# mako443/Text2Pos-CVPR2022

Hardware: AMD Instinct MI355X
Metric: cells+queries encoded/sec and top-k retrieval QPS, 256-pt cells, 12k-cell DB (higher is better)
Workload: dtype f16x3 (fp32 operands split hi+lo into fp16, 3 f16 MFMAs, fp32 accumulate; fp32-class error) for the encoders / f64 MFMA for the ranking

## Files before the change

include/t2p.h:

```cpp
#ifndef T2P_H
#define T2P_H
#include <stddef.h>
#include <stdint.h>

#ifdef __cplusplus
extern "C" {
#endif

#define T2P_ABI_VERSION 32
#define T2P_DEFAULT_CHUNK_OBJECTS 65000
#define T2P_MAX_CHUNK_OBJECTS 65535
#define T2P_TUNING_MASK 0xD
#define T2P_E_ARG (-1)
#define T2P_E_WORKSPACE (-2)
#define T2P_E_UNSUPPORTED (-3)

typedef void* t2p_stream_t;

int t2p_abi_version(void);
const char* t2p_last_error(void);

typedef struct t2p_cell_weights {
    const float* sa_w1[3];
    const float* sa_b1[3];
// ... 230 lines not shown
int t2p_hardest_ranking(const float* scores, int32_t batch, float margin, float* best, int32_t* where, float* d_scores,
                        t2p_stream_t stream);

int t2p_sample_group(const float* xyz, int64_t n_obj, int32_t n_pts, const float* radius_host ,
                     uint8_t* const* fps_idx , uint8_t* const* nbr , uint8_t* const* cnt ,
                     t2p_stream_t stream);
int t2p_group_rows(const float* xyz, int64_t n_obj, int32_t n_pts, const float* radius_host , int32_t self_loops,
                   uint8_t* const* fps_idx , uint16_t* const* rows , uint16_t* const* n_rows ,
                   t2p_stream_t stream);
int t2p_group_rows_shared(const float* xyz, int64_t n_obj, int32_t n_pts, const float* radius_host , int32_t self_loops,
                          int32_t share_mask, uint8_t* const* fps_idx , uint16_t* const* rows ,
                          uint16_t* const* n_rows , t2p_stream_t stream);
int t2p_group_rows_built(const float* xyz, const float* rgb, int64_t n_obj, int32_t n_pts, const float* radius_host ,
                         int32_t self_loops, int32_t share_mask, uint8_t* const* fps_idx , uint16_t* const* rows ,
                         uint16_t* const* n_rows , t2p_stream_t stream);
int t2p_edge_counts(const uint16_t* rows, const uint16_t* n_rows, const int32_t* first_obj, int64_t n_obj, int32_t n_dense,
                    int32_t n_cent, int32_t self_loops, int32_t* counts, t2p_stream_t stream);
int t2p_edge_expand(const uint16_t* rows, const uint16_t* n_rows, const int32_t* first_obj, const int32_t* cent_ptr, int64_t n_obj,
                    int32_t n_dense, int32_t n_cent, int32_t self_loops, int32_t* src, int32_t* dst, t2p_stream_t stream);
int t2p_dedup_rows(const float* xyz, const float* rgb, int64_t n_obj, int32_t n_pts, uint16_t* rows, uint16_t* n_rows,
                   t2p_stream_t stream);
int t2p_knn(const float* x, int32_t dim, const int32_t* seg_ptr, int32_t n_seg, int32_t max_seg_rows, int32_t k,
            int32_t* out_idx, t2p_stream_t stream);
int t2p_gemm(const float* a, int32_t lda, const float* w, const float* bias, float* c, int32_t ldc, int32_t c0,
             int64_t m, int32_t k, int32_t n, int32_t relu, t2p_stream_t stream);
int t2p_gemm_residual(const float* a, int32_t lda, const float* w, const float* bias, float* c, int32_t ldc, int32_t c0,
                      int64_t m, int32_t k, int32_t n, int32_t relu, const float* resid, int32_t ldr, t2p_stream_t stream);
int t2p_gemm_x3(const float* a, int32_t lda, const void* wx, float scale, const float* bias, float* c, int32_t ldc, int32_t c0,
                int64_t m, int32_t k, int32_t n, int32_t relu, const float* resid, int32_t ldr, uint32_t* amax_in,
                t2p_stream_t stream);
// ... 15 lines not shown
```

profiles/tail_rows_census.py:

```python
#!/usr/bin/env python
import argparse
import os
import sys

import numpy as np

sys.path.insert(0, os.path.join(os.path.dirname(os.path.abspath(__file__)), ".."))

RADII = (0.2, 0.3, 0.4)
MAX_NBR = 32


def level(pos: np.ndarray, r: float):
    n_d = pos.shape[0]
    n_c = (n_d + 1) // 2
    r2 = np.float32(r) * np.float32(r)
    mind = np.full(n_d, np.inf, dtype=np.float32)
    fps = np.zeros(n_c, dtype=np.int64)
    cnt = np.zeros(n_c, dtype=np.int64)
    cur = 0
    for c in range(n_c):
        fps[c] = cur
        d = pos - pos[cur]
        d2 = (d[:, 0] * d[:, 0] + d[:, 1] * d[:, 1]) + d[:, 2] * d[:, 2]
        cnt[c] = min(int((d2 < r2).sum()), MAX_NBR)
        mind = np.minimum(mind, d2)
        cur = int(np.argmax(mind))
    return fps, cnt


def dedup_hits(pos: np.ndarray, rgb: np.ndarray, fps: np.ndarray, r: float) -> int:
    key = np.concatenate([pos, rgb], axis=1).view(np.uint32)
    _, first = np.unique(key, axis=0, return_index=True)
    orig = np.zeros(pos.shape[0], dtype=bool)
    orig[first] = True
    r2 = np.float32(r) * np.float32(r)
    kept = 0
    for c in fps:
        d = pos - pos[c]
        d2 = (d[:, 0] * d[:, 0] + d[:, 1] * d[:, 1]) + d[:, 2] * d[:, 2]
        hits = np.flatnonzero(d2 < r2)[:MAX_NBR]
        kept += int(orig[hits].sum())
    return kept
# ... 3 lines not shown
    ap = argparse.ArgumentParser(description=__doc__.split("\n")[0])
    ap.add_argument("--seed", type=int, default=20220002, help="bench.py's object stream")
    ap.add_argument("--objects", type=int, default=3000)
    args = ap.parse_args()
    from importlib import import_module
    S = import_module("text2pos-cvpr2022_amd.synthetic")
    xyz, rgb, _, _ = S.make_objects(args.seed, 0, args.objects)
    n = xyz.shape[0]
    rows = np.zeros(3)
    rows_dedup = 0.0
    with_tail = np.zeros(3)
    tail_cent = np.zeros(3)
    tail_rows = np.zeros(3)
    executed = np.zeros(3)
    cents = np.zeros(3)
    for o in range(n):
        pos = xyz[o].astype(np.float32)
        for l in range(3):
            fps, cnt = level(pos, RADII[l])
            n_c = fps.shape[0]
            tail = (fps == 0) & (np.arange(n_c) > 0)
            all_rows = cnt.sum() + n_c
            t_rows = cnt[tail].sum()
            rows[l] += all_rows
            cents[l] += n_c
            with_tail[l] += tail.any()
            tail_cent[l] += tail.sum()
            tail_rows[l] += t_rows
            executed[l] += all_rows - t_rows + (cnt[0] if tail.any() else 0)
            if l == 0:
                rows_dedup += dedup_hits(pos, rgb[o].astype(np.float32), fps, RADII[0]) + n_c
            pos = pos[fps]
    print(f"{n} objects of seed {args.seed}")
    print("level | rows/object | objects with a tail | tail centroids | tail rows (non-self) | rows/object, tail shared")
    for l in range(3):
        extra = f" ({rows_dedup / n:.0f} after point dedup)" if l == 0 else ""
        print(f"SA{l + 1}   | {rows[l] / n:8.0f}{extra} | {100 * with_tail[l] / n:5.1f} % | {100 * tail_cent[l] / cents[l]:5.1f} % | "
              f"{100 * tail_rows[l] / rows[l]:5.1f} % | {executed[l] / n:8.0f} ({100 * (executed[l] / rows[l] - 1):+.1f} %)")


if __name__ == "__main__":
    main()
```

text2pos-cvpr2022_amd/_lib.py:

```python
import ctypes as C
import os

import torch

_HERE = os.path.dirname(os.path.abspath(__file__))
LIB_PATH = os.environ.get("T2P_LIB") or os.path.join(_HERE, "libt2p_hip.so")
ABI_VERSION = 32

c_float_p = C.POINTER(C.c_float)
c_void = C.c_void_p


class CellWeights(C.Structure):
    _names = (["sa_w1", "sa_b1", "sa_w2", "sa_b2"], ["ga_w1", "ga_b1", "ga_w2", "ga_b2", "lin1_w", "lin1_b", "lin2_w",
              "lin2_b", "pn_w", "pn_b", "col_w1", "col_b1", "col_w2", "col_b2", "pos_w1", "pos_b1", "pos_w2", "pos_b2",
              "merge_w", "merge_b", "g_wp", "g_bp", "g_wq", "g_w2", "g_b2", "lin_w1", "lin_b1", "lin_w2", "lin_b2"])
    _fields_ = ([(n, c_void * 3) for n in _names[0]] + [(n, c_void) for n in _names[1]] +
                [("sa_w2_x3", c_void * 3), ("ga_w2_x3", c_void), ("sa_b2_x3", c_void * 3), ("sa_w2_scale", C.c_float * 3),
                 ("lin1_x3", c_void), ("lin2_x3", c_void), ("merge_x3", c_void), ("pn_x3", c_void), ("g_wp_x3", c_void),
                 ("g_wq_x3", c_void), ("lin1_scale", C.c_float), ("lin2_scale", C.c_float), ("merge_scale", C.c_float),
                 ("pn_scale", C.c_float), ("g_wp_scale", C.c_float), ("g_wq_scale", C.c_float),
                 ("sa_w1_x3", c_void * 3), ("ga_w1_x3", c_void),
                 ("class_embedding", c_void), ("color_embedding", c_void),
                 ("ga_w1_l1", C.c_float), ("ga_b1_absmax", C.c_float), ("sa_wp_l1", C.c_float * 3),
# ... 94 lines not shown
    "t2p_matching_loss_backward": (C.c_int, [c_void, C.c_int64, C.c_int32, C.c_int32, c_void, c_void, C.c_int64, c_void, c_void,
                                             c_void]),
    "t2p_mse_loss_backward": (C.c_int, [c_void, c_void, C.c_int64, c_void, c_void, c_void]),
    "t2p_colsum": (C.c_int, [c_void, C.c_int64, C.c_int32, c_void, c_void]),
    "t2p_profile_enable": (None, [C.c_int]),
    "t2p_profile_report": (C.c_int, [C.c_char_p, C.c_size_t]),
    "t2p_profile_repeat": (None, [C.c_char_p, C.c_int32]),
    "t2p_sample_group": (C.c_int, [c_void, C.c_int64, C.c_int32, c_float_p, C.POINTER(c_void), C.POINTER(c_void),
                                   C.POINTER(c_void), c_void]),
    "t2p_group_rows": (C.c_int, [c_void, C.c_int64, C.c_int32, c_float_p, C.c_int32, C.POINTER(c_void), C.POINTER(c_void),
                                 C.POINTER(c_void), c_void]),
    "t2p_group_rows_shared": (C.c_int, [c_void, C.c_int64, C.c_int32, c_float_p, C.c_int32, C.c_int32, C.POINTER(c_void),
                                        C.POINTER(c_void), C.POINTER(c_void), c_void]),
    "t2p_group_rows_built": (C.c_int, [c_void, c_void, C.c_int64, C.c_int32, c_float_p, C.c_int32, C.c_int32, C.POINTER(c_void),
                                       C.POINTER(c_void), C.POINTER(c_void), c_void]),
    "t2p_edge_counts": (C.c_int, [c_void, c_void, c_void, C.c_int64, C.c_int32, C.c_int32, C.c_int32, c_void, c_void]),
    "t2p_edge_expand": (C.c_int, [c_void, c_void, c_void, c_void, C.c_int64, C.c_int32, C.c_int32, C.c_int32, c_void, c_void, c_void]),
    "t2p_dedup_rows": (C.c_int, [c_void, c_void, C.c_int64, C.c_int32, c_void, c_void, c_void]),
    "t2p_knn": (C.c_int, [c_void, C.c_int32, c_void, C.c_int32, C.c_int32, C.c_int32, c_void, c_void]),
    "t2p_gemm": (C.c_int, [c_void, C.c_int32, c_void, c_void, c_void, C.c_int32, C.c_int32, C.c_int64, C.c_int32,
                           C.c_int32, C.c_int32, c_void]),
    "t2p_rownorm": (C.c_int, [c_void, C.c_int64, C.c_int32, c_void, c_void]),
    "t2p_gemm_residual": (C.c_int, [c_void, C.c_int32, c_void, c_void, c_void, C.c_int32, C.c_int32, C.c_int64, C.c_int32,
                                    C.c_int32, C.c_int32, c_void, C.c_int32, c_void]),
    "t2p_gemm_x3": (C.c_int, [c_void, C.c_int32, c_void, C.c_float, c_void, c_void, C.c_int32, C.c_int32, C.c_int64, C.c_int32,
                              C.c_int32, C.c_int32, c_void, C.c_int32, c_void, c_void]),
    "t2p_gemm_skinny": (C.c_int, [c_void, C.c_int32, c_void, c_void, C.c_int32, C.c_int64, C.c_int32, C.c_int32, c_void]),
    "t2p_linear_wgrad_workspace_bytes": (C.c_size_t, [C.c_int64, C.c_int32, C.c_int32]),
    "t2p_linear_wgrad_f32": (C.c_int, [c_void, C.c_int32, c_void, C.c_int32, c_void, C.c_int32, c_void, C.c_int64, C.c_int32,
                                       C.c_int32, c_void, C.c_size_t, c_void]),
# ... 34 lines not shown
```

text2pos-cvpr2022_amd/csrc/cell_encoder.hip:

```cpp
#include "../../include/t2p.h"
#include "t2p_common.h"

namespace t2p {
namespace {

struct Geo {
    int nd[3], nc[3];
    int gp;
    static constexpr int H[3] = {32, 128, 256};
    static constexpr int C[3] = {64, 128, 256};
    static constexpr int LD[3] = {96, 160, 288};
    explicit Geo(int n_pts) {
        nd[0] = n_pts;
        for (int l = 0; l < 3; l++) {
            nc[l] = (nd[l] + 1) / 2;
            if (l < 2) nd[l + 1] = nc[l];
        }
        gp = 1;
        while (gp < nc[2]) gp *= 2;
    }
    bool specialised(int l) const {
        static constexpr int ND[3] = {256, 128, 64}, NC[3] = {128, 64, 32};
        return nd[l] == ND[l] && nc[l] == NC[l];
    }
// ... 176 lines not shown
    for (int l = 0; l < 3; l++) {
        bp[l].n_rows = gt.n_rows[l];
        bp[l].n_obj = n;
        bp[l].prefix_ws = ws.prefix[l];
        bp[l].bounds_ws = ws.bounds[l];
        bp[l].W_x3 = f16x3() ? W.sa_w2_x3[l] : nullptr;
        bp[l].wp = lds_btab(l) ? W.sa_w1[l] : nullptr;
        bp[l].n_dense = g.nd[l];
        bp[l].n_cent = g.nc[l];
    }
    bp[0].w1 = sa1_points() ? W.sa_w1[0] : nullptr;
    for (int l = 0; l < 3; l++) gt.share_tail[l] = sa_shares_tail_rows(l, Geo::H[l], Geo::C[l], bp[l], cfg.n_pts, cfg.tuning) ? 1 : 0;

    const bool prune_l0 = !(cfg.tuning & 1) && cfg.n_pts == 256;
    gt.mask_l0 = prune_l0 && !(cfg.tuning & 8) && !want_nbr && gt.rows[0] && gt.rows[1] && gt.rows[2] ? 1 : 0;
    T2P_TRY(launch_sample_group(xyz, n, cfg.n_pts, cfg.radius, gt, st));
    if (gt.mask_l0)
        T2P_TRY(launch_build_rows(xyz, rgb, gt.fps_idx[0], n, cfg.n_pts, gt.rows[0], gt.n_rows[0], gt.self_loops, st));
    else if (prune_l0)
        T2P_TRY(launch_dedup_rows(xyz, rgb, n, cfg.n_pts, gt.rows[0], gt.n_rows[0], g.nc[0], st));
    return launch_sa_balance_levels(bp, Geo::H, Geo::C, st);
}

int Chunk::sa_levels(const float* xyz, const float* rgb) const {
    for (int l = 0; l < 3; l++) {
        const int H = Geo::H[l], C = Geo::C[l];
        const int cf = l == 0 ? 3 : Geo::C[l - 1];
        if (l != 0) {
            WsParams p{};
            p.A = ws.F[l - 1];
            p.lda = Geo::LD[l - 1];
            p.k_live = Geo::C[l - 1] + 4;
            p.W = W.sa_w1[l];
// ... 227 lines not shown
        gt.n_dense[l] = g.nd[l];
        gt.n_cent[l] = g.nc[l];
        gt.share_tail[l] = (share_mask >> l) & 1;
    }
    return 0;
}

int group_rows(const char* what, const float* xyz, int64_t n_obj, int32_t n_pts, const float* radius_host, int32_t self_loops,
               int32_t share_mask, uint8_t* const* fps_idx, uint16_t* const* rows, uint16_t* const* n_rows, t2p_stream_t stream) {
    T2P_CHECK_ARG(xyz && radius_host && fps_idx && rows && n_rows, "%s: NULL argument", what);
    T2P_CHECK_ARG((share_mask & ~2) == 0, "%s: share_mask=%#x (bit 1: SA level 2; no other level has a shared form)", what, share_mask);
    T2P_CHECK_ARG(share_mask == 0 || n_pts == 256, "%s: shared lists exist for 256 points per object (n_pts = %d)", what, n_pts);
    GroupTables gt;
    T2P_TRY(fill_group_tables(what, gt, n_pts, self_loops, share_mask, fps_idx, rows, n_rows, nullptr, nullptr));
    return launch_sample_group(xyz, n_obj, n_pts, radius_host, gt, (hipStream_t)stream);
}

}
}

using namespace t2p;

extern "C" {

size_t t2p_encode_cells_workspace_bytes(int64_t n_obj, int64_t n_cells, const t2p_cell_config* cfg) {
    if (cfg == nullptr || n_obj <= 0) return 256;
    int64_t n = default_chunk(*cfg);
    if (n > n_obj) n = n_obj;
    int64_t nb = n_cells < n ? n_cells : n;
    Bump b{nullptr, 0, 0};
// ... 132 lines not shown

int t2p_group_rows(const float* xyz, int64_t n_obj, int32_t n_pts, const float* radius_host, int32_t self_loops,
                   uint8_t* const* fps_idx, uint16_t* const* rows, uint16_t* const* n_rows, t2p_stream_t stream) {
    return group_rows("group_rows", xyz, n_obj, n_pts, radius_host, self_loops, 0, fps_idx, rows, n_rows, stream);
}

int t2p_group_rows_shared(const float* xyz, int64_t n_obj, int32_t n_pts, const float* radius_host, int32_t self_loops,
                          int32_t share_mask, uint8_t* const* fps_idx, uint16_t* const* rows, uint16_t* const* n_rows,
                          t2p_stream_t stream) {
    return group_rows("group_rows_shared", xyz, n_obj, n_pts, radius_host, self_loops, share_mask, fps_idx, rows, n_rows, stream);
}

int t2p_group_rows_built(const float* xyz, const float* rgb, int64_t n_obj, int32_t n_pts, const float* radius_host,
                         int32_t self_loops, int32_t share_mask, uint8_t* const* fps_idx, uint16_t* const* rows,
                         uint16_t* const* n_rows, t2p_stream_t stream) {
    T2P_CHECK_ARG(xyz && rgb && radius_host && fps_idx && rows && n_rows, "group_rows_built: NULL argument");
    T2P_CHECK_ARG(n_obj >= 0, "group_rows_built: negative size");
    T2P_CHECK_ARG((share_mask & ~2) == 0, "group_rows_built: share_mask=%#x (bit 1: SA level 2; no other level has a shared form)", share_mask);
    T2P_CHECK_ARG(n_pts == 256, "group_rows_built: built for 256 points per object (n_pts = %d)", n_pts);
    GroupTables gt;
    T2P_TRY(fill_group_tables("group_rows_built", gt, n_pts, self_loops, share_mask, fps_idx, rows, n_rows, nullptr, nullptr));
    gt.mask_l0 = 1;
    T2P_CHECK_ARG((((uintptr_t)xyz | (uintptr_t)rgb | (uintptr_t)rows[0]) & 15) == 0, "group_rows_built: xyz, rgb and rows[0] must be 16-byte aligned");
    T2P_TRY(launch_sample_group(xyz, n_obj, n_pts, radius_host, gt, (hipStream_t)stream));
    return launch_build_rows(xyz, rgb, gt.fps_idx[0], n_obj, n_pts, gt.rows[0], gt.n_rows[0], gt.self_loops, (hipStream_t)stream);
}

}
```

text2pos-cvpr2022_amd/csrc/sample_group.hip:

```cpp
#include "t2p_common.h"

namespace t2p {

#pragma clang fp contract(off)

namespace {

#ifndef T2P_FPS_PK
#define T2P_FPS_PK 1
#endif

constexpr int kMaxPts = 256;
constexpr int kMaxNbr = 32;

__device__ __forceinline__ float dist2(float ax, float ay, float az, float bx, float by, float bz) {
#pragma clang fp contract(off)
    float dx = ax - bx, dy = ay - by, dz = az - bz;
    float xx = dx * dx, yy = dy * dy, zz = dz * dz;
    float s = xx + yy;
    return s + zz;
}

template <int CTRL>
__device__ __forceinline__ int dpp_i(int v) {
    return __builtin_amdgcn_update_dpp(0, v, CTRL, 0xF, 0xF, true);
// ... 111 lines not shown
    static_assert(!(MASK && SHARE) && (!MASK || PPL == 4), "mask mode: level 0 of the 256-point path");
    const int lane = threadIdx.x;
    const int i0 = MASK ? lane : lane * PPL;
    constexpr int ST = MASK ? 64 : 1;
    float x[PPL], y[PPL], z[PPL];
    uint32_t mind[PPL];
#pragma unroll
    for (int j = 0; j < PPL; j++) {
        x[j] = px[i0 + j * ST];
        y[j] = py[i0 + j * ST];
        z[j] = pz[i0 + j * ST];
        mind[j] = 0x7f800000u;
    }
    int cur = 0;
    int base = 0;
    [[maybe_unused]] bool tail_open = false;
    for (int c = 0; c < n_c; c++) {
        if constexpr (MASK) {
            if (c > 0 && cur == 0) {
                const float x0 = px[0], y0 = py[0], z0 = pz[0];
                for (int t = c + lane; t < n_c; t += 64) {
                    sel[t] = 0;
                    qx[t] = x0;
                    qy[t] = y0;
                    qz[t] = z0;
                }
                break;
            }
        }
        const float cx = px[cur], cy = py[cur], cz = pz[cur];
        if (!MASK && lane == 0) {
            sel[c] = (uint8_t)cur;
            qx[c] = cx;
            qy[c] = cy;
            qz[c] = cz;
        }
        bool tail = false;
        if constexpr (SHARE) {
            tail = c > 0 && cur == 0;
            if (tail && tail_open) {
                if (self_loops && lane == 0) rows_out[(uint32_t)base] = (uint16_t)(((c | 0x80) << 8) | c);
// ... 87 lines not shown
                    }
                }
                cur = 64 * jb + (int)__builtin_ctzll(tie);
            } else {
                const unsigned long long tie = __ballot(bd == mx);
                int jb = PPL - 1;
#pragma unroll
                for (int j = PPL - 2; j >= 0; j--) jb = mind[j] == mx ? j : jb;
                cur = __builtin_amdgcn_readlane(i0 + jb, (int)__builtin_ctzll(tie));
            }
        }
    }
    if constexpr (!MASK) {
        if (lane < 4 && base + lane < n_c * (kMaxNbr + 1)) rows_out[base + lane] = 0xFFFF;
    }
    *n_rows_out = base;
    __syncthreads();
}

__device__ __attribute__((noinline)) void emit_centroid_table(const float* qx, const float* qy, const float* qz, int n_c,
                                                    const float* __restrict__ wp, int H, float* __restrict__ out,
                                                    float* __restrict__ tail, int ld_tail, int tail_col0, int tail_quads,
                                                    int tail_rows) {
    const int lane = threadIdx.x;
    if (tail != nullptr) {
        const int hq = lane % tail_quads;
        for (int c = n_c + lane / tail_quads; c < tail_rows; c += 64 / tail_quads)
            *(f32x4*)(tail + (size_t)c * ld_tail + tail_col0 + hq * 4) =
                hq == 0 ? f32x4{qx[n_c - 1], qy[n_c - 1], qz[n_c - 1], 0.f} : f32x4{0.f, 0.f, 0.f, 0.f};
    }
    if (out == nullptr) {
// ... 77 lines not shown
            }
            guard_publish_bits_above(gt.guard + G_INPUT, in_bits, 0x3f800000u);
        }
        __syncthreads();
        if (gt.A1 != nullptr) {
            const float *w1 = gt.w1, *b1 = gt.b1;
            asm volatile("" : "+s"(w1), "+s"(b1));
            emit_point_table(p0, p0 + kMaxPts, p0 + 2 * kMaxPts, gt.rgb + o * (int64_t)n_pts * 3, n_pts, w1, b1, gt.H1,
                             gt.A1 + o * (int64_t)n_pts * gt.H1);
        }
        float* pin[4][3] = {{p0, p0 + kMaxPts, p0 + 2 * kMaxPts},
                            {p1, p1 + kMaxPts / 2, p1 + kMaxPts},
                            {p2, p2 + kMaxPts / 4, p2 + kMaxPts / 2},
                            {p3, p3 + kMaxPts / 8, p3 + kMaxPts / 4}};
        const float rr[3] = {r0 * r0, r1 * r1, r2 * r2};
#pragma unroll
        for (int l = 0; l < 3; l++) {
            const int n_d = gt.n_dense[l], n_c = gt.n_cent[l];
            if (want_nbr) {
                for (int i = lane; i < n_c * kMaxNbr / 4; i += 64) ((uint32_t*)nbr_lds)[i] = 0u;
            }
            __syncthreads();
            int n_rows = 0;
            uint16_t* g_rows16 = gt.rows[l] ? gt.rows[l] + o * (int64_t)(n_c * (kMaxNbr + 1)) : nullptr;
            if constexpr (FAST) {
                if (l == 0 && MASK)
                    level_fast<4, false, MASK>(pin[l][0], pin[l][1], pin[l][2], n_c, rr[l], sel_lds, pin[l + 1][0], pin[l + 1][1],
                                               pin[l + 1][2], g_rows16, gt.self_loops, &n_rows);
                else if (l == 0)
                    level_fast<4>(pin[l][0], pin[l][1], pin[l][2], n_c, rr[l], sel_lds, pin[l + 1][0], pin[l + 1][1],
                                  pin[l + 1][2], g_rows16, gt.self_loops, &n_rows);
                else if (l == 1 && gt.share_tail[1])
                    level_fast<2, true>(pin[l][0], pin[l][1], pin[l][2], n_c, rr[l], sel_lds, pin[l + 1][0], pin[l + 1][1],
                                        pin[l + 1][2], g_rows16, gt.self_loops, &n_rows, kSaTailCode);
                else if (l == 1)
                    level_fast<2>(pin[l][0], pin[l][1], pin[l][2], n_c, rr[l], sel_lds, pin[l + 1][0], pin[l + 1][1],
                                  pin[l + 1][2], g_rows16, gt.self_loops, &n_rows);
                else
                    level_fast<1>(pin[l][0], pin[l][1], pin[l][2], n_c, rr[l], sel_lds, pin[l + 1][0], pin[l + 1][1],
                                  pin[l + 1][2], g_rows16, gt.self_loops, &n_rows);
            } else if (n_d > 128)
                level<4>(pin[l][0], pin[l][1], pin[l][2], n_d, n_c, rr[l], sel_lds, pin[l + 1][0], pin[l + 1][1],
                         pin[l + 1][2], nbr_lds, cnt_lds, g_rows16, gt.self_loops, &n_rows);
            else if (n_d > 64)
// ... 114 lines not shown
#pragma unroll
    for (int s = 32; s > 0; s >>= 1)
        if (__popcll(w & ((1ull << (p + s)) - 1ull)) < k) p += s;
    return w & ((2ull << p) - 1ull);
}
__device__ __forceinline__ int wave_inclusive_sum(int v) {
    const int lane = threadIdx.x;
#pragma unroll
    for (int d = 1; d < 64; d <<= 1) {
        const int t = __shfl_up(v, d, 64);
        v += lane >= d ? t : 0;
    }
    return v;
}

__global__ __launch_bounds__(64) void k_build_rows(const float* __restrict__ xyz, const float* __restrict__ rgb,
                                                   const uint8_t* __restrict__ fps_idx, int64_t n_obj, uint16_t* rows,
                                                   uint16_t* __restrict__ n_rows, int self_loops) {
    constexpr int NC = kMaxPts / 2, MAXR = NC * (kMaxNbr + 1);
    __shared__ __attribute__((aligned(16))) unsigned char smem[1024 * 4 + 2 * kMaxPts * 3 * 4];
    __shared__ uint8_t rep[kMaxPts];
    uint32_t* const slot = (uint32_t*)smem;
    float* const pxyz = (float*)(smem + 1024 * 4);
    float* const prgb = pxyz + kMaxPts * 3;
    uint16_t* const img = (uint16_t*)smem;
    const int lane = threadIdx.x;
    const int sl = self_loops ? 1 : 0;
    for (int64_t o = blockIdx.x; o < n_obj; o += gridDim.x) {
        repeat_flags(xyz, rgb, o, slot, pxyz, prgb, rep);
        unsigned long long repw[4];
#pragma unroll
        for (int j = 0; j < 4; j++) repw[j] = __ballot(rep[64 * j + lane] != 0);
        uint16_t* const list = rows + o * (int64_t)MAXR;
        const uint8_t* const fo = fps_idx + o * (int64_t)NC;
        const unsigned long long ta = __ballot(lane > 0 && fo[lane] == 0), tb = __ballot(fo[lane + 64] == 0);
        const int t0 = ta != 0 ? (int)__builtin_ctzll(ta) : tb != 0 ? 64 + (int)__builtin_ctzll(tb) : NC;
        const uint4* const mk = (const uint4*)list;
        int n[2], off[2];
        unsigned long long w[2][4];
#pragma unroll
        for (int h = 0; h < 2; h++) {
            const int c = lane + 64 * h;
            const int cm = c < t0 ? c : 0;
            const uint4 lo = mk[2 * cm], hi = mk[2 * cm + 1];
            w[h][0] = (unsigned long long)lo.x | ((unsigned long long)lo.y << 32);
            w[h][1] = (unsigned long long)lo.z | ((unsigned long long)lo.w << 32);
            w[h][2] = (unsigned long long)hi.x | ((unsigned long long)hi.y << 32);
            w[h][3] = (unsigned long long)hi.z | ((unsigned long long)hi.w << 32);
            int left = kMaxNbr;
            n[h] = sl;
#pragma unroll
// ... 21 lines not shown
                unsigned long long x = w[h][j];
                while (x != 0) {
                    img[p++] = (uint16_t)((c << 8) | (64 * j + (int)__builtin_ctzll(x)));
                    x &= x - 1;
                }
            }
            if (sl) img[p] = (uint16_t)(((c | 0x80) << 8) | c);
        }
        if (lane < 12 && total + lane < MAXR) img[total + lane] = 0xFFFF;
        __syncthreads();
        int pieces = (total + 4 + 7) / 8;
        pieces = pieces < MAXR / 8 ? pieces : MAXR / 8;
        for (int i = lane; i < pieces; i += 64) ((uint4*)list)[i] = ((const uint4*)img)[i];
        if (lane == 0) n_rows[o] = (uint16_t)total;
        __syncthreads();
    }
}

}

int launch_dedup_rows(const float* xyz, const float* rgb, int64_t n_obj, int n_pts, uint16_t* rows, uint16_t* n_rows,
                      int n_cent, hipStream_t st) {
    T2P_CHECK_ARG(n_pts == kMaxPts && xyz && rgb && rows && n_rows, "dedup_rows: built for %d points per object", kMaxPts);
    T2P_CHECK_ARG(n_cent > 0 && (n_cent * (kMaxNbr + 1)) % 8 == 0 && ((uintptr_t)rows & 15) == 0,
                  "dedup_rows: the row lists are read 16 bytes at a time: n_cent * 33 must be a multiple of 8 (n_cent = %d)", n_cent);
    if (n_obj == 0) return 0;
    const int64_t grid = n_obj < (int64_t)num_cus() * 32 ? n_obj : (int64_t)num_cus() * 32;
    ProfScope ps_("dedup_rows", st);
    T2P_REPEAT(ps_) hipLaunchKernelGGL(k_dedup_rows, dim3((unsigned)grid), dim3(64), 0, st, xyz, rgb, n_obj, rows, n_rows,
                       n_cent * (kMaxNbr + 1));
    T2P_CHECK_LAUNCH("dedup_rows");
    return 0;
}

int launch_build_rows(const float* xyz, const float* rgb, const uint8_t* fps_idx, int64_t n_obj, int n_pts, uint16_t* rows,
                      uint16_t* n_rows, int self_loops, hipStream_t st) {
    T2P_CHECK_ARG(n_pts == kMaxPts && xyz && rgb && fps_idx && rows && n_rows, "build_rows: built for %d points per object", kMaxPts);
    T2P_CHECK_ARG((((uintptr_t)xyz | (uintptr_t)rgb | (uintptr_t)rows) & 15) == 0, "build_rows: xyz, rgb and rows must be 16-byte aligned");
    if (n_obj == 0) return 0;
    const int64_t grid = n_obj < (int64_t)num_cus() * 64 ? n_obj : (int64_t)num_cus() * 64;
    ProfScope ps_("build_rows", st);
    hipLaunchKernelGGL(k_build_rows, dim3((unsigned)grid), dim3(64), 0, st, xyz, rgb, fps_idx, n_obj, rows, n_rows, self_loops);
    T2P_CHECK_LAUNCH("build_rows");
    return 0;
}

int launch_sample_group(const float* xyz, int64_t n_obj, int n_pts, const float radius[3], GroupTables gt,
                        hipStream_t st) {
    T2P_CHECK_ARG(n_pts >= 8 && n_pts <= kMaxPts, "sample_group: n_pts=%d outside [8,%d]", n_pts, kMaxPts);
    if (n_obj == 0) return 0;
    int64_t grid = n_obj < (int64_t)num_cus() * 64 ? n_obj : (int64_t)num_cus() * 64;
    ProfScope ps_("sample_group", st);
    const bool want_nbr = gt.nbr[0] != nullptr;
    for (int l = 0; l < 3; l++)
        if (gt.B[l] != nullptr)
            T2P_CHECK_ARG(gt.tail[l] == nullptr || gt.H[l] >= 32, "sample_group: tails need H >= 32");
    for (int l = 0; l < 3; l++)
        if (gt.B[l] != nullptr)
            T2P_CHECK_ARG(gt.H[l] % 4 == 0 && gt.H[l] >= 32 && gt.H[l] <= 256 && 64 % (gt.H[l] / 4) == 0 && gt.wp[l],
                          "sample_group: centroid table of level %d: H=%d", l, gt.H[l]);
    if (gt.A1 != nullptr)
        T2P_CHECK_ARG(gt.H1 % 4 == 0 && gt.H1 >= 4 && gt.H1 <= 256 && 64 % (gt.H1 / 4) == 0 && gt.w1 && gt.b1 && gt.rgb,
                      "sample_group: point table: H=%d", gt.H1);
    T2P_CHECK_ARG(!want_nbr || (gt.nbr[1] && gt.nbr[2] && gt.cnt[0] && gt.cnt[1] && gt.cnt[2]),
                  "sample_group: neighbour tables must be given for all levels or none");
    size_t lds = sizeof(float) * 3 * (kMaxPts + kMaxPts / 2 + kMaxPts / 4 + kMaxPts / 8) + kMaxPts / 2;
    if (want_nbr) lds += (kMaxPts / 2) * kMaxNbr + kMaxPts / 2;
    const bool fast = n_pts == kMaxPts && !want_nbr && gt.rows[0] && gt.rows[1] && gt.rows[2] &&
                      gt.n_dense[0] == kMaxPts && gt.n_dense[1] == kMaxPts / 2 && gt.n_dense[2] == kMaxPts / 4;
    T2P_CHECK_ARG(!gt.mask_l0 || (fast && ((uintptr_t)gt.rows[0] & 15) == 0),
                  "sample_group: hit masks (mask_l0) exist for 256 points per object with all row lists wanted, rows 16-byte aligned");
    if (fast && gt.mask_l0)
        T2P_REPEAT(ps_) hipLaunchKernelGGL((k_sample_group<true, true>), dim3((unsigned)grid), dim3(64), lds, st, xyz, n_obj, n_pts,
                           radius[0], radius[1], radius[2], gt);
    else if (fast)
        T2P_REPEAT(ps_) hipLaunchKernelGGL(k_sample_group<true>, dim3((unsigned)grid), dim3(64), lds, st, xyz, n_obj, n_pts, radius[0],
                           radius[1], radius[2], gt);
    else
        hipLaunchKernelGGL(k_sample_group<false>, dim3((unsigned)grid), dim3(64), lds, st, xyz, n_obj, n_pts, radius[0],
                           radius[1], radius[2], gt);
    T2P_CHECK_LAUNCH("sample_group");
    return 0;
}

}
```

text2pos-cvpr2022_amd/csrc/t2p_common.h:

```cpp
#pragma once
#include <hip/hip_runtime.h>
#include <stdint.h>
#include <stdio.h>

namespace t2p {

void set_error(const char* fmt, ...);

#define T2P_E_ARG (-1)
#define T2P_E_WORKSPACE (-2)
#define T2P_E_UNSUPPORTED (-3)

#define T2P_CHECK_ARG(cond, ...)                  \
    do {                                          \
        if (!(cond)) {                            \
            ::t2p::set_error(__VA_ARGS__);        \
            return T2P_E_ARG;                     \
        }                                         \
    } while (0)

#define T2P_CHECK_LAUNCH(name)                                                   \
    do {                                                                         \
        hipError_t e__ = hipGetLastError();                                      \
        if (e__ != hipSuccess) {                                                 \
// ... 120 lines not shown
    int slot;
    hipStream_t st;
    void* ev_end;
    int reps;
};
#define T2P_REPEAT(ps) for (int rep_ = (ps).reps; rep_ > 0; --rep_)

struct GroupTables {
    uint8_t* fps_idx[3];
    uint8_t* nbr[3];
    uint8_t* cnt[3];
    uint16_t* rows[3];
    uint16_t* n_rows[3];
    int self_loops;
    int share_tail[3];
    int mask_l0;
    int n_dense[3];
    int n_cent[3];
    float* B[3];
    const float* wp[3];
    int H[3];
    float* tail[3];
    int ld_tail[3], tail_col0[3];
    int tail_rows[3];
    float* A1;
    const float* w1;
    const float* b1;
    const float* rgb;
    int H1;
    uint32_t* guard;
};
int launch_sample_group(const float* xyz, int64_t n_obj, int n_pts, const float radius[3], GroupTables gt,
                        hipStream_t st);
int launch_dedup_rows(const float* xyz, const float* rgb, int64_t n_obj, int n_pts, uint16_t* rows, uint16_t* n_rows,
                      int n_cent, hipStream_t st);
int launch_build_rows(const float* xyz, const float* rgb, const uint8_t* fps_idx, int64_t n_obj, int n_pts, uint16_t* rows,
                      uint16_t* n_rows, int self_loops, hipStream_t st);

int launch_rownorm(const float* in, int ld_in, int64_t n_rows, int dim, float* out, int ld_out, int col0,
                   hipStream_t st);
int launch_gather_rownorm(const float* table, const int32_t* idx, int64_t n_rows, int dim, float* out, int ld_out,
                          int col0, hipStream_t st);
int launch_segmax(const float* in, int dim, const int32_t* seg_ptr, int n_seg, float* out, int mean,
                  hipStream_t st);
int launch_knn(const float* x, int dim, const int32_t* seg_ptr, int n_seg, int max_seg_rows, int k,
               int32_t* out_idx, hipStream_t st);
int launch_mlp3_norm(const float* in3, int64_t n_rows, const float* w1, const float* b1, const float* w2,
                     const float* b2, int D, float* out, int ld_out, int col0, hipStream_t st);
int launch_pack_objects(const float* raw_xyz, const float* raw_rgb, const int32_t* obj_ptr, const int32_t* sample_idx,
                        const float* rot, int64_t n_obj, int n_pts, float* xyz, float* rgb, float* center, float* mean_rgb,
                        hipStream_t st);
int launch_pack_scene(const float* raw_xyz, const float* raw_rgb, const int32_t* obj_ptr, const int32_t* obj_id, const uint64_t* key,
// ... 157 lines not shown
```

text2pos-cvpr2022_amd/ops.py:

```python
import ctypes as C
import os
from typing import Dict, Optional

import numpy as np
import torch

from . import _lib as L

_workspaces: Dict[tuple, torch.Tensor] = {}


def _stream(device) -> C.c_void_p:
    return C.c_void_p(torch.cuda.current_stream(device).cuda_stream)


def _ptr(t: Optional[torch.Tensor]) -> C.c_void_p:
    return C.c_void_p(0 if t is None else t.data_ptr())


def _need(t: torch.Tensor, name: str, dtype, ndim=None, device=None):
    if not isinstance(t, torch.Tensor):
        raise RuntimeError(f"{name}: expected a torch.Tensor, got {type(t).__name__}")
    if not t.is_cuda:
        raise RuntimeError(f"{name}: must live on the GPU (got device {t.device}); there is no CPU path")
# ... 185 lines not shown
    return out


def group_rows(xyz: torch.Tensor, radius=(0.2, 0.3, 0.4), self_loops: bool = True, share_mask: int = 0):
    _need(xyz, "xyz", torch.float32, 3)
    dev = xyz.device
    n_obj, n_pts, three = xyz.shape
    if three != 3:
        raise RuntimeError(f"xyz: last dimension must be 3, got {three}")
    out, arr = _level_tables(n_obj, n_pts, dev, ("fps_idx", "rows", "n_rows"))
    L.check(L.lib().t2p_group_rows_shared(_ptr(xyz), n_obj, n_pts, _radius(radius), int(bool(self_loops)), int(share_mask),
                                          arr["fps_idx"], arr["rows"], arr["n_rows"], _stream(dev)), "t2p_group_rows_shared")
    return out


def group_rows_built(xyz: torch.Tensor, rgb: torch.Tensor, radius=(0.2, 0.3, 0.4), self_loops: bool = True, share_mask: int = 0):
    _need(xyz, "xyz", torch.float32, 3)
    _need(rgb, "rgb", torch.float32, 3, xyz.device)
    dev = xyz.device
    n_obj, n_pts, three = xyz.shape
    if three != 3 or tuple(rgb.shape) != tuple(xyz.shape):
        raise RuntimeError(f"group_rows_built: xyz and rgb must both be [n_obj, n_pts, 3], got {tuple(xyz.shape)} and {tuple(rgb.shape)}")
    out, arr = _level_tables(n_obj, n_pts, dev, ("fps_idx", "rows", "n_rows"))
    L.check(L.lib().t2p_group_rows_built(_ptr(xyz), _ptr(rgb), n_obj, n_pts, _radius(radius), int(bool(self_loops)), int(share_mask),
                                         arr["fps_idx"], arr["rows"], arr["n_rows"], _stream(dev)), "t2p_group_rows_built")
    return out


def dedup_rows(xyz: torch.Tensor, rgb: torch.Tensor, rows: torch.Tensor, n_rows: torch.Tensor):
    _need(xyz, "xyz", torch.float32, 3)
    _need(rgb, "rgb", torch.float32, 3, xyz.device)
    _need(rows, "rows", torch.int16, 2, xyz.device)
    _need(n_rows, "n_rows", torch.int16, 1, xyz.device)
    n_obj, n_pts = xyz.shape[0], xyz.shape[1]
    if rows.shape[0] != n_obj or rows.shape[1] != ((n_pts + 1) // 2) * 33 or n_rows.numel() != n_obj:
        raise RuntimeError("dedup_rows: inconsistent shapes")
    L.check(L.lib().t2p_dedup_rows(_ptr(xyz), _ptr(rgb), n_obj, n_pts, _ptr(rows), _ptr(n_rows), _stream(xyz.device)),
            "t2p_dedup_rows")


# ... 822 lines not shown
```

Baseline: 158,100.

## Derive SA2/SA3 FPS as prefix of SA1 and build their rows in build_rows

In the mask_l0 plan, the SA2 and SA3 farthest-point selections become the identity prefix of the SA1 centroids, up to the first tail index. The sample_group kernel therefore skips the FPS and ball query for levels 2 and 3. Those levels' neighbour row lists are now built inside k_build_rows from the already-gathered centroid coordinates. Optionally, hits on duplicate dense points beyond the prefix are dropped. This removes two serial FPS passes and separate ball queries, but it adds work and register pressure to build_rows, which now uses launch_bounds(64,4), and it relies on the prefix equivalence holding for the tail-repeat structure.

```diff
diff --git a/include/t2p.h b/include/t2p.h
--- a/include/t2p.h
+++ b/include/t2p.h
@@ -268,6 +268,9 @@
 int t2p_group_rows_built(const float* xyz, const float* rgb, int64_t n_obj, int32_t n_pts, const float* radius_host ,
                          int32_t self_loops, int32_t share_mask, uint8_t* const* fps_idx , uint16_t* const* rows ,
                          uint16_t* const* n_rows , t2p_stream_t stream);
+int t2p_group_rows_pruned(const float* xyz, const float* rgb, int64_t n_obj, int32_t n_pts, const float* radius_host ,
+                          int32_t self_loops, int32_t share_mask, uint8_t* const* fps_idx , uint16_t* const* rows ,
+                          uint16_t* const* n_rows , t2p_stream_t stream);
 int t2p_edge_counts(const uint16_t* rows, const uint16_t* n_rows, const int32_t* first_obj, int64_t n_obj, int32_t n_dense,
                     int32_t n_cent, int32_t self_loops, int32_t* counts, t2p_stream_t stream);
 int t2p_edge_expand(const uint16_t* rows, const uint16_t* n_rows, const int32_t* first_obj, const int32_t* cent_ptr, int64_t n_obj,
diff --git a/profiles/tail_rows_census.py b/profiles/tail_rows_census.py
--- a/profiles/tail_rows_census.py
+++ b/profiles/tail_rows_census.py
@@ -27,6 +27,21 @@
         mind = np.minimum(mind, d2)
         cur = int(np.argmax(mind))
     return fps, cnt
+
+
+def capped_hits(pos: np.ndarray, fps: np.ndarray, r: float):
+    r2 = np.float32(r) * np.float32(r)
+    out = []
+    for c in fps:
+        d = pos - pos[c]
+        d2 = (d[:, 0] * d[:, 0] + d[:, 1] * d[:, 1]) + d[:, 2] * d[:, 2]
+        out.append(np.flatnonzero(d2 < r2)[:MAX_NBR])
+    return out
+
+
+def first_tail(fps: np.ndarray) -> int:
+    t = np.flatnonzero((fps == 0) & (np.arange(len(fps)) > 0))
+    return int(t[0]) if len(t) else len(fps)
 
 
 def dedup_hits(pos: np.ndarray, rgb: np.ndarray, fps: np.ndarray, r: float) -> int:
@@ -60,6 +75,8 @@
     tail_rows = np.zeros(3)
     executed = np.zeros(3)
     cents = np.zeros(3)
+    pruned = np.zeros(3)
+    with_dup = np.zeros(3)
     for o in range(n):
         pos = xyz[o].astype(np.float32)
         for l in range(3):
@@ -76,13 +93,25 @@
             executed[l] += all_rows - t_rows + (cnt[0] if tail.any() else 0)
             if l == 0:
                 rows_dedup += dedup_hits(pos, rgb[o].astype(np.float32), fps, RADII[0]) + n_c
+                k1 = first_tail(fps)
+                pruned[0] += all_rows
+            else:
+                k_prev = min(k1, pos.shape[0])
+                hits = capped_hits(pos, fps, RADII[l])
+                shared = l == 1 and tail.any()
+                listed = [c for c in range(n_c) if not (shared and tail[c])] + ([first_tail(fps)] if shared else [])
+                pruned[l] += sum(int((hits[c] < k_prev).sum()) for c in listed) + n_c
+                with_dup[l] += k_prev < pos.shape[0]
             pos = pos[fps]
     print(f"{n} objects of seed {args.seed}")
-    print("level | rows/object | objects with a tail | tail centroids | tail rows (non-self) | rows/object, tail shared")
+    print("level | rows/object | objects with a tail | tail centroids | tail rows (non-self) | rows/object, tail shared | "
+          "rows/object, duplicate sources dropped | objects with repeated dense points")
     for l in range(3):
         extra = f" ({rows_dedup / n:.0f} after point dedup)" if l == 0 else ""
         print(f"SA{l + 1}   | {rows[l] / n:8.0f}{extra} | {100 * with_tail[l] / n:5.1f} % | {100 * tail_cent[l] / cents[l]:5.1f} % | "
-              f"{100 * tail_rows[l] / rows[l]:5.1f} % | {executed[l] / n:8.0f} ({100 * (executed[l] / rows[l] - 1):+.1f} %)")
+              f"{100 * tail_rows[l] / rows[l]:5.1f} % | {executed[l] / n:8.0f} ({100 * (executed[l] / rows[l] - 1):+.1f} %) | "
+              + (f"{pruned[l] / n:8.0f} ({100 * (pruned[l] / (executed[l] if l == 1 else rows[l]) - 1):+.1f} %) | {100 * with_dup[l] / n:5.1f} %"
+                 if l else "       - |     -"))
 
 
 if __name__ == "__main__":
diff --git a/text2pos-cvpr2022_amd/_lib.py b/text2pos-cvpr2022_amd/_lib.py
--- a/text2pos-cvpr2022_amd/_lib.py
+++ b/text2pos-cvpr2022_amd/_lib.py
@@ -132,6 +132,8 @@
                                         C.POINTER(c_void), C.POINTER(c_void), c_void]),
     "t2p_group_rows_built": (C.c_int, [c_void, c_void, C.c_int64, C.c_int32, c_float_p, C.c_int32, C.c_int32, C.POINTER(c_void),
                                        C.POINTER(c_void), C.POINTER(c_void), c_void]),
+    "t2p_group_rows_pruned": (C.c_int, [c_void, c_void, C.c_int64, C.c_int32, c_float_p, C.c_int32, C.c_int32, C.POINTER(c_void),
+                                        C.POINTER(c_void), C.POINTER(c_void), c_void]),
     "t2p_edge_counts": (C.c_int, [c_void, c_void, c_void, C.c_int64, C.c_int32, C.c_int32, C.c_int32, c_void, c_void]),
     "t2p_edge_expand": (C.c_int, [c_void, c_void, c_void, c_void, C.c_int64, C.c_int32, C.c_int32, C.c_int32, c_void, c_void, c_void]),
     "t2p_dedup_rows": (C.c_int, [c_void, c_void, C.c_int64, C.c_int32, c_void, c_void, c_void]),
diff --git a/text2pos-cvpr2022_amd/csrc/cell_encoder.hip b/text2pos-cvpr2022_amd/csrc/cell_encoder.hip
--- a/text2pos-cvpr2022_amd/csrc/cell_encoder.hip
+++ b/text2pos-cvpr2022_amd/csrc/cell_encoder.hip
@@ -214,9 +214,10 @@
 
     const bool prune_l0 = !(cfg.tuning & 1) && cfg.n_pts == 256;
     gt.mask_l0 = prune_l0 && !(cfg.tuning & 8) && !want_nbr && gt.rows[0] && gt.rows[1] && gt.rows[2] ? 1 : 0;
+    gt.prune_dup[1] = gt.prune_dup[2] = gt.mask_l0 && !(cfg.tuning & 4) && !cfg.self_loops ? 1 : 0;
     T2P_TRY(launch_sample_group(xyz, n, cfg.n_pts, cfg.radius, gt, st));
     if (gt.mask_l0)
-        T2P_TRY(launch_build_rows(xyz, rgb, gt.fps_idx[0], n, cfg.n_pts, gt.rows[0], gt.n_rows[0], gt.self_loops, st));
+        T2P_TRY(launch_build_rows(xyz, rgb, n, cfg.n_pts, cfg.radius, gt, st));
     else if (prune_l0)
         T2P_TRY(launch_dedup_rows(xyz, rgb, n, cfg.n_pts, gt.rows[0], gt.n_rows[0], g.nc[0], st));
     return launch_sa_balance_levels(bp, Geo::H, Geo::C, st);
@@ -474,6 +475,23 @@
     GroupTables gt;
     T2P_TRY(fill_group_tables(what, gt, n_pts, self_loops, share_mask, fps_idx, rows, n_rows, nullptr, nullptr));
     return launch_sample_group(xyz, n_obj, n_pts, radius_host, gt, (hipStream_t)stream);
+}
+
+int group_rows_built(const char* what, const float* xyz, const float* rgb, int64_t n_obj, int32_t n_pts, const float* radius_host,
+                     int32_t self_loops, int32_t share_mask, int prune_dup, uint8_t* const* fps_idx, uint16_t* const* rows,
+                     uint16_t* const* n_rows, t2p_stream_t stream) {
+    T2P_CHECK_ARG(xyz && rgb && radius_host && fps_idx && rows && n_rows, "%s: NULL argument", what);
+    T2P_CHECK_ARG(n_obj >= 0, "%s: negative size", what);
+    T2P_CHECK_ARG((share_mask & ~2) == 0, "%s: share_mask=%#x (bit 1: SA level 2; no other level has a shared form)", what, share_mask);
+    T2P_CHECK_ARG(n_pts == 256, "%s: built for 256 points per object (n_pts = %d)", what, n_pts);
+    GroupTables gt;
+    T2P_TRY(fill_group_tables(what, gt, n_pts, self_loops, share_mask, fps_idx, rows, n_rows, nullptr, nullptr));
+    gt.mask_l0 = 1;
+    gt.prune_dup[1] = gt.prune_dup[2] = prune_dup;
+    T2P_CHECK_ARG((((uintptr_t)xyz | (uintptr_t)rgb | (uintptr_t)rows[0] | (uintptr_t)rows[1] | (uintptr_t)rows[2]) & 15) == 0,
+                  "%s: xyz, rgb and rows must be 16-byte aligned", what);
+    T2P_TRY(launch_sample_group(xyz, n_obj, n_pts, radius_host, gt, (hipStream_t)stream));
+    return launch_build_rows(xyz, rgb, n_obj, n_pts, radius_host, gt, (hipStream_t)stream);
 }
 
 }
@@ -636,16 +654,13 @@
 int t2p_group_rows_built(const float* xyz, const float* rgb, int64_t n_obj, int32_t n_pts, const float* radius_host,
                          int32_t self_loops, int32_t share_mask, uint8_t* const* fps_idx, uint16_t* const* rows,
                          uint16_t* const* n_rows, t2p_stream_t stream) {
-    T2P_CHECK_ARG(xyz && rgb && radius_host && fps_idx && rows && n_rows, "group_rows_built: NULL argument");
-    T2P_CHECK_ARG(n_obj >= 0, "group_rows_built: negative size");
-    T2P_CHECK_ARG((share_mask & ~2) == 0, "group_rows_built: share_mask=%#x (bit 1: SA level 2; no other level has a shared form)", share_mask);
-    T2P_CHECK_ARG(n_pts == 256, "group_rows_built: built for 256 points per object (n_pts = %d)", n_pts);
-    GroupTables gt;
-    T2P_TRY(fill_group_tables("group_rows_built", gt, n_pts, self_loops, share_mask, fps_idx, rows, n_rows, nullptr, nullptr));
-    gt.mask_l0 = 1;
-    T2P_CHECK_ARG((((uintptr_t)xyz | (uintptr_t)rgb | (uintptr_t)rows[0]) & 15) == 0, "group_rows_built: xyz, rgb and rows[0] must be 16-byte aligned");
-    T2P_TRY(launch_sample_group(xyz, n_obj, n_pts, radius_host, gt, (hipStream_t)stream));
-    return launch_build_rows(xyz, rgb, gt.fps_idx[0], n_obj, n_pts, gt.rows[0], gt.n_rows[0], gt.self_loops, (hipStream_t)stream);
-}
-
-}
+    return group_rows_built("group_rows_built", xyz, rgb, n_obj, n_pts, radius_host, self_loops, share_mask, 0, fps_idx, rows, n_rows, stream);
+}
+
+int t2p_group_rows_pruned(const float* xyz, const float* rgb, int64_t n_obj, int32_t n_pts, const float* radius_host,
+                          int32_t self_loops, int32_t share_mask, uint8_t* const* fps_idx, uint16_t* const* rows,
+                          uint16_t* const* n_rows, t2p_stream_t stream) {
+    return group_rows_built("group_rows_pruned", xyz, rgb, n_obj, n_pts, radius_host, self_loops, share_mask, 1, fps_idx, rows, n_rows, stream);
+}
+
+}
diff --git a/text2pos-cvpr2022_amd/csrc/sample_group.hip b/text2pos-cvpr2022_amd/csrc/sample_group.hip
--- a/text2pos-cvpr2022_amd/csrc/sample_group.hip
+++ b/text2pos-cvpr2022_amd/csrc/sample_group.hip
@@ -9,6 +9,13 @@
 #ifndef T2P_FPS_PK
 #define T2P_FPS_PK 1
 #endif
+#ifndef T2P_PREFIX_FPS
+#define T2P_PREFIX_FPS 1
+#endif
+#ifndef T2P_PRUNE_ROWS
+#define T2P_PRUNE_ROWS T2P_PREFIX_FPS
+#endif
+static_assert(T2P_PREFIX_FPS || !T2P_PRUNE_ROWS, "T2P_PRUNE_ROWS needs T2P_PREFIX_FPS");
 
 constexpr int kMaxPts = 256;
 constexpr int kMaxNbr = 32;
@@ -150,6 +157,7 @@
     }
     int cur = 0;
     int base = 0;
+    [[maybe_unused]] int k1 = n_c;
     [[maybe_unused]] bool tail_open = false;
     for (int c = 0; c < n_c; c++) {
         if constexpr (MASK) {
@@ -161,6 +169,7 @@
                     qy[t] = y0;
                     qz[t] = z0;
                 }
+                k1 = c;
                 break;
             }
         }
@@ -278,7 +287,10 @@
     if constexpr (!MASK) {
         if (lane < 4 && base + lane < n_c * (kMaxNbr + 1)) rows_out[base + lane] = 0xFFFF;
     }
-    *n_rows_out = base;
+    if constexpr (MASK)
+        *n_rows_out = k1;
+    else
+        *n_rows_out = base;
     __syncthreads();
 }
 
@@ -386,9 +398,25 @@
                             {p2, p2 + kMaxPts / 4, p2 + kMaxPts / 2},
                             {p3, p3 + kMaxPts / 8, p3 + kMaxPts / 4}};
         const float rr[3] = {r0 * r0, r1 * r1, r2 * r2};
+        [[maybe_unused]] int k1 = kMaxPts / 2;
 #pragma unroll
         for (int l = 0; l < 3; l++) {
             const int n_d = gt.n_dense[l], n_c = gt.n_cent[l];
+            if (FAST && MASK && T2P_PREFIX_FPS && l > 0) {
+                uint8_t* g_sel = gt.fps_idx[l] + o * (int64_t)n_c;
+                for (int i = lane; i < n_c; i += 64) g_sel[i] = (uint8_t)(i < k1 ? i : 0);
+                if (gt.B[l] != nullptr || gt.tail[l] != nullptr) {
+                    const float* wpl = gt.wp[l];
+                    asm volatile("" : "+s"(wpl));
+                    const int t_rows = gt.tail_rows[l] > n_c ? gt.tail_rows[l] : n_c;
+                    emit_centroid_table(pin[1][0], pin[1][1], pin[1][2], n_c, wpl, gt.H[l],
+                                        gt.B[l] ? gt.B[l] + o * (int64_t)n_c * gt.H[l] : nullptr,
+                                        gt.tail[l] ? gt.tail[l] + o * (int64_t)t_rows * gt.ld_tail[l] : nullptr, gt.ld_tail[l],
+                                        gt.tail_col0[l], l == 2 ? 8 : 1, t_rows);
+                }
+                if (l == 2) __syncthreads();
+                continue;
+            }
             if (want_nbr) {
                 for (int i = lane; i < n_c * kMaxNbr / 4; i += 64) ((uint32_t*)nbr_lds)[i] = 0u;
             }
@@ -396,10 +424,11 @@
             int n_rows = 0;
             uint16_t* g_rows16 = gt.rows[l] ? gt.rows[l] + o * (int64_t)(n_c * (kMaxNbr + 1)) : nullptr;
             if constexpr (FAST) {
-                if (l == 0 && MASK)
+                if (l == 0 && MASK) {
                     level_fast<4, false, MASK>(pin[l][0], pin[l][1], pin[l][2], n_c, rr[l], sel_lds, pin[l + 1][0], pin[l + 1][1],
                                                pin[l + 1][2], g_rows16, gt.self_loops, &n_rows);
-                else if (l == 0)
+                    k1 = n_rows;
+                } else if (l == 0)
                     level_fast<4>(pin[l][0], pin[l][1], pin[l][2], n_c, rr[l], sel_lds, pin[l + 1][0], pin[l + 1][1],
                                   pin[l + 1][2], g_rows16, gt.self_loops, &n_rows);
                 else if (l == 1 && gt.share_tail[1])
@@ -544,9 +573,49 @@
     return v;
 }
 
-__global__ __launch_bounds__(64) void k_build_rows(const float* __restrict__ xyz, const float* __restrict__ rgb,
+struct BuildUpper {
+    uint16_t* rows[2];
+    uint16_t* n_rows[2];
+    float rr[2];
+    int share;
+    int prune[2];
+};
+
+template <int NW>
+__device__ __forceinline__ void store_lane_lists(uint16_t* img, uint16_t* list, uint16_t* n_rows_o, int max_rows, bool active,
+                                                 const uint32_t (&w)[NW], bool hits, int tag, int sl) {
+    const int lane = threadIdx.x;
+    int n = sl;
+#pragma unroll
+    for (int i = 0; i < NW; i++) n += hits ? __popc(w[i]) : 0;
+    n = active ? n : 0;
+    const int s = wave_inclusive_sum(n);
+    const int total = __builtin_amdgcn_readlane(s, 63);
+    int p = s - n;
+    if (active) {
+        const uint32_t t = (uint32_t)tag << 8;
+#pragma unroll
+        for (int i = 0; i < NW; i++) {
+            uint32_t x = hits ? w[i] : 0u;
+            while (x != 0) {
+                img[p++] = (uint16_t)(t | (uint32_t)(32 * i + __builtin_ctz(x)));
+                x &= x - 1;
+            }
+        }
+        if (sl) img[p] = (uint16_t)(((lane | 0x80) << 8) | lane);
+    }
+    if (lane < 12 && total + lane < max_rows) img[total + lane] = 0xFFFF;
+    __syncthreads();
+    int pieces = (total + 4 + 7) / 8;
+    pieces = pieces < max_rows / 8 ? pieces : max_rows / 8;
+    for (int i = lane; i < pieces; i += 64) ((uint4*)list)[i] = ((const uint4*)img)[i];
+    if (lane == 0) *n_rows_o = (uint16_t)total;
+    __syncthreads();
+}
+
+__global__ __launch_bounds__(64, 4) void k_build_rows(const float* __restrict__ xyz, const float* __restrict__ rgb,
                                                    const uint8_t* __restrict__ fps_idx, int64_t n_obj, uint16_t* rows,
-                                                   uint16_t* __restrict__ n_rows, int self_loops) {
+                                                   uint16_t* __restrict__ n_rows, int self_loops, BuildUpper up) {
     constexpr int NC = kMaxPts / 2, MAXR = NC * (kMaxNbr + 1);
     __shared__ __attribute__((aligned(16))) unsigned char smem[1024 * 4 + 2 * kMaxPts * 3 * 4];
     __shared__ uint8_t rep[kMaxPts];
@@ -565,6 +634,16 @@
         const uint8_t* const fo = fps_idx + o * (int64_t)NC;
         const unsigned long long ta = __ballot(lane > 0 && fo[lane] == 0), tb = __ballot(fo[lane + 64] == 0);
         const int t0 = ta != 0 ? (int)__builtin_ctzll(ta) : tb != 0 ? 64 + (int)__builtin_ctzll(tb) : NC;
+        float* const q = (float*)(smem + MAXR * 2);
+        if (T2P_PREFIX_FPS) {
+#pragma unroll
+            for (int h = 0; h < 2; h++) {
+                const int c = lane + 64 * h, i = fo[c];
+                q[c] = pxyz[i * 3];
+                q[NC + c] = pxyz[i * 3 + 1];
+                q[2 * NC + c] = pxyz[i * 3 + 2];
+            }
+        }
         const uint4* const mk = (const uint4*)list;
         int n[2], off[2];
         unsigned long long w[2][4];
@@ -616,6 +695,61 @@
         for (int i = lane; i < pieces; i += 64) ((uint4*)list)[i] = ((const uint4*)img)[i];
         if (lane == 0) n_rows[o] = (uint16_t)total;
         __syncthreads();
+        if (T2P_PREFIX_FPS) {
+            constexpr int NC1 = kMaxPts / 4, NC2 = kMaxPts / 8;
+            const int e1 = t0, e2 = t0 < NC1 ? t0 : NC1;
+            typedef float f32x2 __attribute__((ext_vector_type(2)));
+            const float cx = q[lane], cy = q[NC + lane], cz = q[2 * NC + lane];
+            const f32x2 c2x = {cx, cx}, c2y = {cy, cy}, c2z = {cz, cz};
+            const float rr1 = up.rr[0], rr2 = up.rr[1];
+            uint32_t w1[4] = {0u, 0u, 0u, 0u}, w2[2] = {0u, 0u};
+#pragma unroll
+            for (int b = 0; b < 4; b++) {
+                if (32 * b < e1) {
+#pragma unroll
+                    for (int u = 0; u < 32; u += 2) {
+#pragma clang fp contract(off)
+                        const int j = 32 * b + u;
+                        const f32x2 dx = *(const f32x2*)(q + j) - c2x, dy = *(const f32x2*)(q + NC + j) - c2y,
+                                    dz = *(const f32x2*)(q + 2 * NC + j) - c2z;
+                        const f32x2 xx = dx * dx, yy = dy * dy, zz = dz * dz;
+                        const f32x2 sxy = xx + yy;
+                        const f32x2 dd = sxy + zz;
+                        w1[b] |= (dd[0] < rr1 ? 1u << u : 0u) | (dd[1] < rr1 ? 2u << u : 0u);
+                        if (b < 2) w2[b] |= (dd[0] < rr2 ? 1u << u : 0u) | (dd[1] < rr2 ? 2u << u : 0u);
+                    }
+                }
+            }
+            const uint32_t v1 = !up.prune[0] && (w1[0] & 1u) ? ~0u : 0u, v2 = !up.prune[1] && (w2[0] & 1u) ? ~0u : 0u;
+#pragma unroll
+            for (int b = 0; b < 4; b++) {
+                const int live = e1 - 32 * b;
+                const uint32_t keep = live >= 32 ? ~0u : live <= 0 ? 0u : (1u << live) - 1u;
+                w1[b] = (w1[b] & keep) | (v1 & ~keep);
+                if (b < 2) {
+                    const int live2 = e2 - 32 * b;
+                    const uint32_t keep2 = live2 >= 32 ? ~0u : live2 <= 0 ? 0u : (1u << live2) - 1u;
+                    w2[b] = (w2[b] & keep2) | (v2 & ~keep2);
+                }
+            }
+            unsigned long long m1a = (unsigned long long)w1[0] | ((unsigned long long)w1[1] << 32);
+            unsigned long long m1b = (unsigned long long)w1[2] | ((unsigned long long)w1[3] << 32);
+            unsigned long long m2 = (unsigned long long)w2[0] | ((unsigned long long)w2[1] << 32);
+            int pc = __popcll(m1a);
+            if (pc > kMaxNbr) {
+                m1a = lowest_set_bits(m1a, kMaxNbr);
+                pc = kMaxNbr;
+            }
+            if (__popcll(m1b) > kMaxNbr - pc) m1b = lowest_set_bits(m1b, kMaxNbr - pc);
+            if (__popcll(m2) > kMaxNbr) m2 = lowest_set_bits(m2, kMaxNbr);
+            const uint32_t l1[4] = {(uint32_t)m1a, (uint32_t)(m1a >> 32), (uint32_t)m1b, (uint32_t)(m1b >> 32)};
+            const uint32_t l2[2] = {(uint32_t)m2, (uint32_t)(m2 >> 32)};
+            const bool tail = up.share && lane >= t0;
+            store_lane_lists(img, up.rows[0] + o * (int64_t)(NC1 * (kMaxNbr + 1)), up.n_rows[0] + o, NC1 * (kMaxNbr + 1), true, l1,
+                             !tail || lane == t0, tail ? kSaTailCode : lane, sl);
+            store_lane_lists(img, up.rows[1] + o * (int64_t)(NC2 * (kMaxNbr + 1)), up.n_rows[1] + o, NC2 * (kMaxNbr + 1), lane < NC2, l2,
+                             true, lane, sl);
+        }
     }
 }
 
@@ -635,14 +769,29 @@
     return 0;
 }
 
-int launch_build_rows(const float* xyz, const float* rgb, const uint8_t* fps_idx, int64_t n_obj, int n_pts, uint16_t* rows,
-                      uint16_t* n_rows, int self_loops, hipStream_t st) {
+int launch_build_rows(const float* xyz, const float* rgb, int64_t n_obj, int n_pts, const float radius[3], const GroupTables& gt,
+                      hipStream_t st) {
+    const uint8_t* fps_idx = gt.fps_idx[0];
+    uint16_t *rows = gt.rows[0], *n_rows = gt.n_rows[0];
+    const int self_loops = gt.self_loops;
     T2P_CHECK_ARG(n_pts == kMaxPts && xyz && rgb && fps_idx && rows && n_rows, "build_rows: built for %d points per object", kMaxPts);
     T2P_CHECK_ARG((((uintptr_t)xyz | (uintptr_t)rgb | (uintptr_t)rows) & 15) == 0, "build_rows: xyz, rgb and rows must be 16-byte aligned");
+    BuildUpper up{};
+    if (T2P_PREFIX_FPS) {
+        T2P_CHECK_ARG(gt.rows[1] && gt.rows[2] && gt.n_rows[1] && gt.n_rows[2] && (((uintptr_t)gt.rows[1] | (uintptr_t)gt.rows[2]) & 15) == 0,
+                      "build_rows: the row lists of levels 2 and 3 are written here, 16 bytes at a time");
+        for (int l = 1; l < 3; l++) {
+            up.rows[l - 1] = gt.rows[l];
+            up.n_rows[l - 1] = gt.n_rows[l];
+            up.rr[l - 1] = radius[l] * radius[l];
+            up.prune[l - 1] = T2P_PRUNE_ROWS && gt.prune_dup[l] ? 1 : 0;
+        }
+        up.share = gt.share_tail[1];
+    }
     if (n_obj == 0) return 0;
     const int64_t grid = n_obj < (int64_t)num_cus() * 64 ? n_obj : (int64_t)num_cus() * 64;
     ProfScope ps_("build_rows", st);
-    hipLaunchKernelGGL(k_build_rows, dim3((unsigned)grid), dim3(64), 0, st, xyz, rgb, fps_idx, n_obj, rows, n_rows, self_loops);
+    hipLaunchKernelGGL(k_build_rows, dim3((unsigned)grid), dim3(64), 0, st, xyz, rgb, fps_idx, n_obj, rows, n_rows, self_loops, up);
     T2P_CHECK_LAUNCH("build_rows");
     return 0;
 }
@@ -672,6 +821,8 @@
                       gt.n_dense[0] == kMaxPts && gt.n_dense[1] == kMaxPts / 2 && gt.n_dense[2] == kMaxPts / 4;
     T2P_CHECK_ARG(!gt.mask_l0 || (fast && ((uintptr_t)gt.rows[0] & 15) == 0),
                   "sample_group: hit masks (mask_l0) exist for 256 points per object with all row lists wanted, rows 16-byte aligned");
+    T2P_CHECK_ARG(!(gt.prune_dup[0] || gt.prune_dup[1] || gt.prune_dup[2]) || (gt.mask_l0 && !gt.prune_dup[0]),
+                  "sample_group: prune_dup exists for levels 2 and 3 of the hit-mask plan (mask_l0)");
     if (fast && gt.mask_l0)
         T2P_REPEAT(ps_) hipLaunchKernelGGL((k_sample_group<true, true>), dim3((unsigned)grid), dim3(64), lds, st, xyz, n_obj, n_pts,
                            radius[0], radius[1], radius[2], gt);
diff --git a/text2pos-cvpr2022_amd/csrc/t2p_common.h b/text2pos-cvpr2022_amd/csrc/t2p_common.h
--- a/text2pos-cvpr2022_amd/csrc/t2p_common.h
+++ b/text2pos-cvpr2022_amd/csrc/t2p_common.h
@@ -158,6 +158,7 @@
     uint16_t* n_rows[3];
     int self_loops;
     int share_tail[3];
+    int prune_dup[3];
     int mask_l0;
     int n_dense[3];
     int n_cent[3];
@@ -178,8 +179,8 @@
                         hipStream_t st);
 int launch_dedup_rows(const float* xyz, const float* rgb, int64_t n_obj, int n_pts, uint16_t* rows, uint16_t* n_rows,
                       int n_cent, hipStream_t st);
-int launch_build_rows(const float* xyz, const float* rgb, const uint8_t* fps_idx, int64_t n_obj, int n_pts, uint16_t* rows,
-                      uint16_t* n_rows, int self_loops, hipStream_t st);
+int launch_build_rows(const float* xyz, const float* rgb, int64_t n_obj, int n_pts, const float radius[3], const GroupTables& gt,
+                      hipStream_t st);
 
 int launch_rownorm(const float* in, int ld_in, int64_t n_rows, int dim, float* out, int ld_out, int col0,
                    hipStream_t st);
diff --git a/text2pos-cvpr2022_amd/ops.py b/text2pos-cvpr2022_amd/ops.py
--- a/text2pos-cvpr2022_amd/ops.py
+++ b/text2pos-cvpr2022_amd/ops.py
@@ -223,7 +223,8 @@
     return out
 
 
-def group_rows_built(xyz: torch.Tensor, rgb: torch.Tensor, radius=(0.2, 0.3, 0.4), self_loops: bool = True, share_mask: int = 0):
+def group_rows_built(xyz: torch.Tensor, rgb: torch.Tensor, radius=(0.2, 0.3, 0.4), self_loops: bool = True, share_mask: int = 0,
+                     prune_dup: bool = False):
     _need(xyz, "xyz", torch.float32, 3)
     _need(rgb, "rgb", torch.float32, 3, xyz.device)
     dev = xyz.device
@@ -231,8 +232,9 @@
     if three != 3 or tuple(rgb.shape) != tuple(xyz.shape):
         raise RuntimeError(f"group_rows_built: xyz and rgb must both be [n_obj, n_pts, 3], got {tuple(xyz.shape)} and {tuple(rgb.shape)}")
     out, arr = _level_tables(n_obj, n_pts, dev, ("fps_idx", "rows", "n_rows"))
-    L.check(L.lib().t2p_group_rows_built(_ptr(xyz), _ptr(rgb), n_obj, n_pts, _radius(radius), int(bool(self_loops)), int(share_mask),
-                                         arr["fps_idx"], arr["rows"], arr["n_rows"], _stream(dev)), "t2p_group_rows_built")
+    name = "t2p_group_rows_pruned" if prune_dup else "t2p_group_rows_built"
+    L.check(getattr(L.lib(), name)(_ptr(xyz), _ptr(rgb), n_obj, n_pts, _radius(radius), int(bool(self_loops)), int(share_mask),
+                                   arr["fps_idx"], arr["rows"], arr["n_rows"], _stream(dev)), name)
     return out
 
 
```

Measured after the change: 159,800, median of 6. 1.1% higher.
